# tnwei/waternet

Measured on NVIDIA H100. Metric: images/sec at 1080p batch16 (preprocess + gated-fusion forward, uint8 in -> uint8 out), higher is better.
Workload: dtype bf16 + fp8 corrections (v = hi + lo: hi x hi in bf16, both correction terms of the heavy layers as one e4m3 MMA; fp32 accumulate; 3-term bf16 elsewhere)

## Files before the change

### waternet_b200/csrc/umma_conv.cuh

```cuda
#pragma once

#include <cuda.h>
#include <cuda_bf16.h>

#include "common.cuh"
#include "wgmma_ops.cuh"

namespace wn {

__device__ __forceinline__ uint32_t smem_u32(const void* p) {
  return (uint32_t)__cvta_generic_to_shared(p);
}
__device__ __forceinline__ void mbar_init(uint64_t* bar, uint32_t count) {
  asm volatile("mbarrier.init.shared::cta.b64 [%0], %1;" ::"r"(smem_u32(bar)), "r"(count));
}
__device__ __forceinline__ void mbar_wait(uint64_t* bar, uint32_t parity) {
  for (uint32_t it = 0; it < (1u << 26); it++) {
    uint32_t done;
    asm volatile(
        "{\n\t.reg .pred p;\n\t"
        "mbarrier.try_wait.parity.shared::cta.b64 p, [%1], %2;\n\t"
        "selp.u32 %0, 1, 0, p;\n\t}"
        : "=r"(done)
        : "r"(smem_u32(bar)), "r"(parity)
        : "memory");
    if (done) return;
  }
  __trap();
}
__device__ __forceinline__ void mbar_arrive(uint64_t* bar) {
  asm volatile("mbarrier.arrive.shared::cta.b64 _, [%0];" ::"r"(smem_u32(bar)) : "memory");
}
__device__ __forceinline__ void mbar_expect_tx(uint64_t* bar, uint32_t bytes) {
  asm volatile("mbarrier.arrive.expect_tx.shared::cta.b64 _, [%0], %1;" ::"r"(smem_u32(bar)), "r"(bytes)
               : "memory");
}
__device__ __forceinline__ void tma_load_5d(void* dst, const CUtensorMap* tmap, uint64_t* bar, int c0,
                                            int c1, int c2, int c3, int c4) {
  asm volatile(
      "cp.async.bulk.tensor.5d.shared::cluster.global.mbarrier::complete_tx::bytes [%0], [%1, {%3, %4, %5, %6, %7}], [%2];"
      ::"r"(smem_u32(dst)), "l"(tmap), "r"(smem_u32(bar)), "r"(c0), "r"(c1), "r"(c2), "r"(c3), "r"(c4)
      : "memory");
}
__device__ __forceinline__ void bulk_load(void* dst, const void* src, uint32_t bytes, uint64_t* bar) {
  asm volatile(
      "cp.async.bulk.shared::cluster.global.mbarrier::complete_tx::bytes [%0], [%1], %2, [%3];" ::"r"(
          smem_u32(dst)),
      "l"(src), "r"(bytes), "r"(smem_u32(bar))
      : "memory");
}
__device__ __forceinline__ uint64_t make_desc(uint32_t addr, uint32_t lbo, uint32_t sbo) {
  return (uint64_t)((addr >> 4) & 0x3fff) | ((uint64_t)((lbo >> 4) & 0x3fff) << 16) |
         ((uint64_t)((sbo >> 4) & 0x3fff) << 32);
}
__device__ __forceinline__ void wg_fence() { asm volatile("wgmma.fence.sync.aligned;" ::: "memory"); }
__device__ __forceinline__ void wg_commit() { asm volatile("wgmma.commit_group.sync.aligned;" ::: "memory"); }
template <int PENDING>
__device__ __forceinline__ void wg_wait() { asm volatile("wgmma.wait_group.sync.aligned %0;" ::"n"(PENDING) : "memory"); }
__device__ __forceinline__ void wg_bar(int id) { asm volatile("bar.sync %0, 128;" ::"r"(id) : "memory"); }
__device__ __forceinline__ uint32_t pack_e4m3x4(float f0, float f1, float f2, float f3) {
  uint16_t lo, hi;
  asm("cvt.rn.satfinite.e4m3x2.f32 %0, %1, %2;" : "=h"(lo) : "f"(f1), "f"(f0));
  asm("cvt.rn.satfinite.e4m3x2.f32 %0, %1, %2;" : "=h"(hi) : "f"(f3), "f"(f2));
  return (uint32_t)lo | ((uint32_t)hi << 16);
}
__device__ __forceinline__ uint16_t pack_e4m3x2(float f0, float f1) {
  uint16_t v;
  asm("cvt.rn.satfinite.e4m3x2.f32 %0, %1, %2;" : "=h"(v) : "f"(f1), "f"(f0));
  return v;
}

enum Epilogue { kEpiAct = 0, kEpiSigmoid = 1, kEpiGate = 2, kEpiDgrad = 3 };

constexpr int kTileW = 8, kTileH = 16;
constexpr int kThreads = 320;
constexpr int kWarpA = 8, kWarpB = 9;
constexpr int kConsumerWarps = 8;
constexpr int kStageLd = 36;

constexpr int kFmtIn8 = 1, kFmtOut8 = 2;
template <int KS, int CIN_PAD, int NPAD, int CONCAT = 0, int NBLK = 1, int TPS = 1, int FMT = 0>
struct UmmaCfg {
  static constexpr bool F8IN = (FMT & kFmtIn8) != 0;
  static constexpr bool DUAL = CONCAT != 0;
  static constexpr int HALO_W = kTileW + KS - 1, HALO_H = kTileH + KS - 1;
  static constexpr int NCHUNK = CIN_PAD / 16;
  static constexpr int PLANE_BYTES = HALO_W * HALO_H * 16;
  static constexpr int A_STAGE = (4 * PLANE_BYTES + 1023) / 1024 * 1024;
  static constexpr int B_TAP = NPAD * 64;
  static constexpr int B_STAGE = TPS * B_TAP;
  static_assert((KS * KS) % TPS == 0, "taps per weight stage must divide the filter");
  static constexpr int NSTAGE_PER_CHUNK = KS * KS / TPS;
  static constexpr int STAGING = 2 * 64 * kStageLd * 4;
  static constexpr int BUDGET = 227 * 1024 - 1024 - 2048 - STAGING;
  static constexpr int NA_WANT = NCHUNK == 1 ? 2 : KS == 1 ? 6 : 3;
  static constexpr int NB_FIT = (BUDGET - NA_WANT * A_STAGE) / B_STAGE;
  static constexpr int NB = NB_FIT > 8 ? 8 : NB_FIT < 2 ? 2 : NB_FIT;
  static constexpr int NA_FIT = (BUDGET - NB * B_STAGE) / A_STAGE;
  static constexpr int NA = NA_FIT > NA_WANT ? NA_WANT : NA_FIT;
  static_assert(!F8IN || !CONCAT, "fp8 corrections: the [hi | second part] weight layout");
  static constexpr int CPB = NCHUNK / NBLK;
  static constexpr int BLK_COLS = DUAL ? 2 * NPAD : NPAD;
  static constexpr int COLS = NBLK * BLK_COLS;
  static constexpr int ACC = COLS / 2;
  static constexpr int ACC8 = F8IN ? ACC : 1;
  static constexpr int SMEM_BYTES = NA * A_STAGE + NB * B_STAGE + STAGING + 2048 + 1024;
  static_assert(NA >= 1, "halo tile does not fit in shared memory");
  static_assert(NCHUNK % NBLK == 0, "chunks must split evenly over the diagonal blocks");
  static_assert(NPAD % 16 == 0 && (DUAL ? 2 : 1) * NPAD <= 256, "invalid wgmma N");
  static_assert(ACC + (F8IN ? ACC8 : 0) <= 128, "accumulators do not fit in registers");
};

struct ActDst {
  uint4* base;
  int planes_half;
};

struct ConvArgs {
  const uint8_t* wpk;
  const float* bias;
  int N, H, W;
  int in_planes_half;
  int tiles_x, tiles_y;
  ActDst dst0, dst1;
  int split_c;
  int cout;
  float* out_f32;
  const float* cm;
  uint8_t* out_u8;
  const int* skip_lo;
  int a_hi_only;
  float* refined_out;
  const uint4* mask_base;
  int mask_planes_half;
  const float* f8_scale;
  int* f8_overflow;
  const int* run_if;
  int tiled;
  long long win0;
  TileGeom tiles;
  const RaggedWindow* rwin;
};

__device__ __forceinline__ uint32_t pack_bf16x2(__nv_bfloat16 a, __nv_bfloat16 b) {
  return (uint32_t)__bfloat16_as_ushort(a) | ((uint32_t)__bfloat16_as_ushort(b) << 16);
}
__device__ __forceinline__ void split_bf16x2(float f0, float f1, uint32_t& hi, uint32_t& lo) {
  const __nv_bfloat162 h = __floats2bfloat162_rn(f0, f1);
  hi = *reinterpret_cast<const uint32_t*>(&h);
  const float h0 = __uint_as_float(hi << 16), h1 = __uint_as_float(hi & 0xffff0000u);
  const __nv_bfloat162 l = __floats2bfloat162_rn(f0 - h0, f1 - h1);
  lo = *reinterpret_cast<const uint32_t*>(&l);
}

template <int EPI, bool OUT8, bool RAG = false>
__device__ __forceinline__ void epilogue16(const ConvArgs& g, const float* s_bias, const float* f, int ch, int n,
                                           int gx, int gy, bool valid = true) {
  const size_t hw = (size_t)g.H * g.W;
  const size_t pix = (size_t)gy * g.W + gx;
  if constexpr (EPI == kEpiAct || EPI == kEpiDgrad) {
    if (ch >= g.cout) return;
    if constexpr (OUT8) {
      uint32_t hi[8], l8[4], h8[4];
      float vmax = 0.f;
#pragma unroll
      for (int j = 0; j < 16; j += 4) {
        float v[4], r[4];
#pragma unroll
        for (int t = 0; t < 4; t++) {
          v[t] = fmaxf(f[j + t] + s_bias[ch + j + t], 0.f);
          if constexpr (RAG) v[t] = valid ? v[t] : 0.f;
          vmax = fmaxf(vmax, v[t]);
        }
#pragma unroll
        for (int t = 0; t < 4; t += 2) {
          const __nv_bfloat162 h = __floats2bfloat162_rn(v[t], v[t + 1]);
          const uint32_t hb = *reinterpret_cast<const uint32_t*>(&h);
          hi[(j + t) >> 1] = hb;
          r[t] = (v[t] - __uint_as_float(hb << 16)) * 512.f;
          r[t + 1] = (v[t + 1] - __uint_as_float(hb & 0xffff0000u)) * 512.f;
        }
        l8[j >> 2] = pack_e4m3x4(r[0], r[1], r[2], r[3]);
        h8[j >> 2] = pack_e4m3x4(v[0], v[1], v[2], v[3]);
      }
      if (!(vmax <= 448.f) && g.f8_overflow) atomicOr(g.f8_overflow, 1);
      const bool second = ch >= g.split_c;
      const ActDst& d = second ? g.dst1 : g.dst0;
      const int chl = second ? ch - g.split_c : ch;
      uint4* p_hi = d.base + ((size_t)n * 2 * d.planes_half + (chl >> 3)) * hw + pix;
      uint4* p_f8 = d.base + ((size_t)n * 2 * d.planes_half + d.planes_half + 2 * (chl >> 4)) * hw + pix;
      p_hi[0] = make_uint4(hi[0], hi[1], hi[2], hi[3]);
      p_hi[hw] = make_uint4(hi[4], hi[5], hi[6], hi[7]);
      p_f8[0] = make_uint4(l8[0], l8[1], l8[2], l8[3]);
      p_f8[hw] = make_uint4(h8[0], h8[1], h8[2], h8[3]);
    } else {
#pragma unroll
      for (int q = 0; q < 16; q += 8) {
        const int c = ch + q;
        if (c >= g.cout) break;
        uint32_t hi[4], lo[4];
        uint32_t mask[4] = {0xffffffffu, 0xffffffffu, 0xffffffffu, 0xffffffffu};
        if constexpr (EPI == kEpiDgrad) {
          if (g.mask_base) {
            const uint4 m = g.mask_base[((size_t)n * 2 * g.mask_planes_half + (c >> 3)) * hw + pix];
            mask[0] = m.x; mask[1] = m.y; mask[2] = m.z; mask[3] = m.w;
          }
        }
#pragma unroll
        for (int j = 0; j < 8; j += 2) {
          float f0, f1;
          if constexpr (EPI == kEpiDgrad) {
            f0 = (mask[j >> 1] & 0x0000ffffu) ? f[q + j] : 0.f;
            f1 = (mask[j >> 1] & 0xffff0000u) ? f[q + j + 1] : 0.f;
          } else {
            f0 = fmaxf(f[q + j] + s_bias[c + j], 0.f);
            f1 = fmaxf(f[q + j + 1] + s_bias[c + j + 1], 0.f);
            if constexpr (RAG) {
              f0 = valid ? f0 : 0.f;
              f1 = valid ? f1 : 0.f;
            }
          }
          split_bf16x2(f0, f1, hi[j >> 1], lo[j >> 1]);
        }
        const bool second = c >= g.split_c;
        const ActDst& d = second ? g.dst1 : g.dst0;
        const int plane = (second ? c - g.split_c : c) >> 3;
        uint4* p_hi = d.base + ((size_t)n * 2 * d.planes_half + plane) * hw + pix;
        p_hi[0] = make_uint4(hi[0], hi[1], hi[2], hi[3]);
        p_hi[(size_t)d.planes_half * hw] = make_uint4(lo[0], lo[1], lo[2], lo[3]);
      }
    }
  } else {
    if (ch != 0) return;
    const size_t o = (size_t)n * 3 * hw + pix;
    if constexpr (EPI == kEpiSigmoid) {
#pragma unroll
      for (int c = 0; c < 3; c++) g.out_f32[o + c * hw] = 1.0f / (1.0f + expf(-(f[c] + s_bias[c])));
    } else {
      float r[9];
#pragma unroll
      for (int j = 0; j < 9; j++) r[j] = fmaxf(f[j] + s_bias[j], 0.f);
      if (g.refined_out) {
#pragma unroll
        for (int j = 0; j < 9; j++) g.refined_out[(size_t)n * 9 * hw + pix + j * hw] = r[j];
      }
      if (g.cm) {
        const float c0 = g.cm[o], c1 = g.cm[o + hw], c2 = g.cm[o + 2 * hw];
        float v[3];
#pragma unroll
        for (int c = 0; c < 3; c++)
          v[c] = __fadd_rn(__fadd_rn(__fmul_rn(r[c], c0), __fmul_rn(r[3 + c], c1)), __fmul_rn(r[6 + c], c2));
        size_t oo = o, ohw = hw, o8 = ((size_t)n * hw + pix) * 3;
        float* out_f32 = g.out_f32;
        uint8_t* out_u8 = g.out_u8;
        if constexpr (RAG) {
          const RaggedWindow& t = g.rwin[n];
          const int y = t.ys + gy, x = t.xs + gx;
          if (y < t.ky0 || y >= t.ky1 || x < t.kx0 || x >= t.kx1) return;
          ohw = (size_t)t.H * t.W;
          oo = (size_t)y * t.W + x;
          o8 = oo * 3;
          out_f32 = t.out_f32;
          out_u8 = t.out_u8;
        } else if (g.tiled) {
          const TileWindow t = tile_window(g.tiles, g.win0 + n);
          const int y = t.ys + gy, x = t.xs + gx;
          if (y < t.ky0 || y >= t.ky1 || x < t.kx0 || x >= t.kx1) return;
          ohw = (size_t)g.tiles.H * g.tiles.W;
          const size_t ipix = (size_t)y * g.tiles.W + x;
          oo = (size_t)t.img * 3 * ohw + ipix;
          o8 = ((size_t)t.img * ohw + ipix) * 3;
        }
        if (out_f32) {
#pragma unroll
          for (int c = 0; c < 3; c++) out_f32[oo + c * ohw] = v[c];
        }
        if (out_u8) {
          uint8_t* q = out_u8 + o8;
#pragma unroll
          for (int c = 0; c < 3; c++) q[c] = (uint8_t)(int)__fmul_rn(fminf(fmaxf(v[c], 0.0f), 1.0f), 255.0f);
        }
      }
    }
  }
}

template <int KS, int CIN_PAD, int NPAD, int EPI, int CONCAT, int NBLK, int TPS, int FMT = 0, bool RAG = false>
__global__ void __launch_bounds__(kThreads, 1)
conv_umma_kernel(const __grid_constant__ CUtensorMap tmap_in, const ConvArgs g) {
  using C = UmmaCfg<KS, CIN_PAD, NPAD, CONCAT, NBLK, TPS, FMT>;
  constexpr bool F8IN = C::F8IN, DUAL = C::DUAL, OUT8 = (FMT & kFmtOut8) != 0;
  static_assert(!OUT8 || EPI == kEpiAct, "fp8 planes are written by the activation epilogue only");
  static_assert(!RAG || EPI == kEpiAct || EPI == kEpiGate, "ragged passes mask activations and store the gate");
  if (g.run_if != nullptr && *reinterpret_cast<const volatile int*>(g.run_if) == 0) return;
  extern __shared__ uint8_t smem_raw[];
  uint8_t* smem = reinterpret_cast<uint8_t*>((reinterpret_cast<uintptr_t>(smem_raw) + 1023) & ~(uintptr_t)1023);
  uint8_t* a_stages = smem;
  uint8_t* b_stages = smem + C::NA * C::A_STAGE;
  float* staging = reinterpret_cast<float*>(b_stages + C::NB * C::B_STAGE);
  uint8_t* tail = reinterpret_cast<uint8_t*>(staging) + C::STAGING;
  uint64_t* a_full = reinterpret_cast<uint64_t*>(tail);
  uint64_t* a_empty = a_full + C::NA;
  uint64_t* b_full = a_empty + C::NA;
  uint64_t* b_empty = b_full + C::NB;
  float* s_bias = reinterpret_cast<float*>(tail + 512);
  static_assert((2 * 6 + 2 * 8) * 8 <= 512 && NBLK * NPAD * 4 <= 2048 - 512, "barrier / bias area");

  const int tid = threadIdx.x, warp = tid >> 5, lane = tid & 31;
  const int num_tiles = g.tiles_x * g.tiles_y * g.N;
  if (tid == 0) {
    for (int i = 0; i < C::NA; i++) { mbar_init(&a_full[i], 1); mbar_init(&a_empty[i], kConsumerWarps); }
    for (int i = 0; i < C::NB; i++) { mbar_init(&b_full[i], 1); mbar_init(&b_empty[i], kConsumerWarps); }
    asm volatile("fence.mbarrier_init.release.cluster;" ::: "memory");
  }
  for (int i = tid; i < NBLK * NPAD; i += kThreads) s_bias[i] = g.bias[i];
  __syncthreads();

  if (warp == kWarpA) {
    if (lane == 0) {
      int stage = 0;
      uint32_t phase = 0;
      for (int tile = blockIdx.x; tile < num_tiles; tile += gridDim.x) {
        const int n = tile / (g.tiles_x * g.tiles_y);
        const int rem = tile - n * g.tiles_x * g.tiles_y;
        const int ty = rem / g.tiles_x, tx = rem - ty * g.tiles_x;
        const int x0 = tx * kTileW - KS / 2, y0 = ty * kTileH - KS / 2;
        for (int c = 0; c < C::NCHUNK; c++) {
          mbar_wait(&a_empty[stage], phase ^ 1);
          uint8_t* dst = a_stages + stage * C::A_STAGE;
          mbar_expect_tx(&a_full[stage], (g.a_hi_only ? 2 : 4) * C::PLANE_BYTES);
          tma_load_5d(dst, &tmap_in, &a_full[stage], 0, x0, y0, 2 * c, n);
          if (!g.a_hi_only)
            tma_load_5d(dst + 2 * C::PLANE_BYTES, &tmap_in, &a_full[stage], 0, x0, y0, g.in_planes_half + 2 * c, n);
          if (++stage == C::NA) { stage = 0; phase ^= 1; }
        }
      }
    }
    return;
  }
  if (warp == kWarpB) {
    if (lane == 0) {
      int stage = 0;
      uint32_t phase = 0;
      for (int tile = blockIdx.x; tile < num_tiles; tile += gridDim.x) {
        for (int it = 0; it < C::NCHUNK * C::NSTAGE_PER_CHUNK; it++) {
          mbar_wait(&b_empty[stage], phase ^ 1);
          mbar_expect_tx(&b_full[stage], C::B_STAGE);
          bulk_load(b_stages + stage * C::B_STAGE, g.wpk + (size_t)it * C::B_STAGE, C::B_STAGE, &b_full[stage]);
          if (++stage == C::NB) { stage = 0; phase ^= 1; }
        }
      }
    }
    return;
  }

  const int wg = warp >> 2, wtid = tid & 127;
  const bool skip_lo = (g.skip_lo != nullptr && *g.skip_lo != 0) || g.a_hi_only;
  const float dscale = F8IN ? *g.f8_scale : 1.f;
  constexpr uint32_t kSboA = C::HALO_W * 16;
  constexpr uint32_t kLboB = (CONCAT ? 2 * NPAD : NPAD) * 16;
  float acc[C::ACC], acc8[C::ACC8];
  int astage = 0, bstage = 0, pend_a = -1, pend_b = -1;
  uint32_t aphase = 0, bphase = 0;
  auto release = [&]() {
    if (lane == 0) {
      if (pend_b >= 0) mbar_arrive(&b_empty[pend_b]);
      if (pend_a >= 0) mbar_arrive(&a_empty[pend_a]);
    }
    pend_a = pend_b = -1;
  };
  for (int tile = blockIdx.x; tile < num_tiles; tile += gridDim.x) {
#pragma unroll
    for (int i = 0; i < C::ACC; i++) acc[i] = 0.f;
#pragma unroll
    for (int i = 0; i < C::ACC8; i++) acc8[i] = 0.f;
#pragma unroll
    for (int c = 0; c < C::NCHUNK; c++) {
      mbar_wait(&a_full[astage], aphase);
      const uint32_t a_base = smem_u32(a_stages + astage * C::A_STAGE) + (uint32_t)(wg * 8 * C::HALO_W * 16);
      const int blk = NBLK > 1 ? c / C::CPB : 0;
      for (int tg = 0; tg < C::NSTAGE_PER_CHUNK; tg++) {
        mbar_wait(&b_full[bstage], bphase);
        const uint32_t b_base = smem_u32(b_stages + bstage * C::B_STAGE);
        wg_fence();
#pragma unroll
        for (int t = 0; t < TPS; t++) {
          const int tap = tg * TPS + t;
          const int ky = tap / KS, kx = tap - ky * KS;
          const uint32_t a_tap = a_base + (uint32_t)((ky * C::HALO_W + kx) * 16);
          const uint32_t b_tap = b_base + (uint32_t)(t * C::B_TAP);
          const uint64_t a_hi = make_desc(a_tap, C::PLANE_BYTES, kSboA);
          const uint64_t a_lo = make_desc(a_tap + 2 * C::PLANE_BYTES, C::PLANE_BYTES, kSboA);
#pragma unroll
          for (int b = 0; b < NBLK; b++) {
            if (NBLK > 1 && b != blk) continue;
            float* d = acc + b * C::BLK_COLS / 2;
            if constexpr (F8IN) {
              wgmma_bf16<NPAD>(d, a_hi, make_desc(b_tap, NPAD * 16, 128));
              wgmma_e4m3<NPAD>(acc8 + b * C::BLK_COLS / 2, a_lo, make_desc(b_tap + NPAD * 32, NPAD * 16, 128));
            } else if constexpr (CONCAT) {
              wgmma_bf16<2 * NPAD>(d, a_hi, make_desc(b_tap, kLboB, 128));
              if (!skip_lo) wgmma_bf16<NPAD>(d, a_lo, make_desc(b_tap, kLboB, 128));
            } else {
              wgmma_bf16<NPAD>(d, a_hi, make_desc(b_tap, kLboB, 128));
              if (!skip_lo) wgmma_bf16<NPAD>(d, a_lo, make_desc(b_tap, kLboB, 128));
              wgmma_bf16<NPAD>(d, a_hi, make_desc(b_tap + 2 * NPAD * 16, kLboB, 128));
            }
          }
        }
        wg_commit();
        wg_wait<1>();
        release();
        pend_b = bstage;
        if (tg == C::NSTAGE_PER_CHUNK - 1) pend_a = astage;
        if (++bstage == C::NB) { bstage = 0; bphase ^= 1; }
      }
      if (++astage == C::NA) { astage = 0; aphase ^= 1; }
    }
    wg_wait<0>();
    release();

    const int n = tile / (g.tiles_x * g.tiles_y);
    const int rem = tile - n * g.tiles_x * g.tiles_y;
    const int ty = rem / g.tiles_x, tx = rem - ty * g.tiles_x;
    float* stg = staging + wg * 64 * kStageLd;
    const int frow = (warp & 3) * 16 + (lane >> 2), fcol = (lane & 3) * 2;
    const int r = wtid & 63, half = wtid >> 6;
    const int m = wg * 64 + r;
    const int gx = tx * kTileW + (m & 7), gy = ty * kTileH + (m >> 3);
    const bool inside = gx < g.W && gy < g.H;
    bool valid = true;
    if constexpr (RAG) valid = gx < g.rwin[n].vw && gy < g.rwin[n].vh;
    constexpr int NCH = NBLK * NPAD;
#pragma unroll
    for (int ch0 = 0; ch0 < NCH; ch0 += 32) {
#pragma unroll
      for (int j = 0; j < 4; j++) {
        const int ch = ch0 + 8 * j;
        if (ch < NCH) {
          const int col = NBLK > 1 ? (ch / NPAD) * C::BLK_COLS + ch % NPAD : ch;
          float v[4];
#pragma unroll
          for (int k = 0; k < 4; k++) {
            v[k] = acc[col / 2 + k];
            if constexpr (DUAL) v[k] += acc[(col + NPAD) / 2 + k];
            if constexpr (F8IN) v[k] = (v[k] + acc8[col / 2 + k]) * dscale;
          }
          float* s = stg + frow * kStageLd + 8 * j + fcol;
          *reinterpret_cast<float2*>(s) = make_float2(v[0], v[1]);
          *reinterpret_cast<float2*>(s + 8 * kStageLd) = make_float2(v[2], v[3]);
        }
      }
      wg_bar(1 + wg);
      const int cb = ch0 + 16 * half;
      if (cb < NCH && inside) {
        float f[16];
        const float4* s = reinterpret_cast<const float4*>(stg + r * kStageLd + 16 * half);
#pragma unroll
        for (int q = 0; q < 4; q++) {
          const float4 x = s[q];
          f[4 * q] = x.x; f[4 * q + 1] = x.y; f[4 * q + 2] = x.z; f[4 * q + 3] = x.w;
        }
        epilogue16<EPI, OUT8, RAG>(g, s_bias, f, cb, n, gx, gy, valid);
      }
      wg_bar(1 + wg);
    }
  }
}

static __global__ void scatter_weights_kernel(const float* __restrict__ src, float* __restrict__ dense, int co, int ci,
                                       int kk, int cinpad, int row_off, int split, int base0, int base1,
                                       float divisor) {
  const int total = co * ci * kk;
  for (int i = blockIdx.x * blockDim.x + threadIdx.x; i < total; i += gridDim.x * blockDim.x) {
    int t = i % kk;
    int c = (i / kk) % ci;
    int o = i / (kk * ci);
    int cd = c < split ? base0 + c : base1 + (c - split);
    dense[((size_t)(row_off + o) * cinpad + cd) * kk + t] = __fdiv_rn(src[i], divisor);
  }
}
static __global__ void scatter_bias_kernel(const float* __restrict__ src, float* __restrict__ dst, int co, int row_off) {
  for (int i = blockIdx.x * blockDim.x + threadIdx.x; i < co; i += gridDim.x * blockDim.x) dst[row_off + i] = src[i];
}
static __global__ void pack_stages_kernel(const float* __restrict__ dense, __nv_bfloat16* __restrict__ out, int npad,
                                   int cinpad, int kk, int concat, int nblk) {
  const int nchunk = cinpad / 16, cpb = nchunk / nblk;
  const size_t total = (size_t)nchunk * kk * 2 * 2 * npad * 8;
  for (size_t i = (size_t)blockIdx.x * blockDim.x + threadIdx.x; i < total; i += (size_t)gridDim.x * blockDim.x) {
    int e = (int)(i % 8);
    size_t r = i / 8;
    int k8, split, nrow;
    if (concat) {
      int row2 = (int)(r % (2 * npad)); r /= 2 * npad;
      k8 = (int)(r % 2); r /= 2;
      split = row2 >= npad;
      nrow = row2 - split * npad;
    } else {
      nrow = (int)(r % npad); r /= npad;
      k8 = (int)(r % 2); r /= 2;
      split = (int)(r % 2); r /= 2;
    }
    int tap = (int)(r % kk);
    int chunk = (int)(r / kk);
    int cin = chunk * 16 + k8 * 8 + e;
    int row = (chunk / cpb) * npad + nrow;
    float w = dense[((size_t)row * cinpad + cin) * kk + tap];
    __nv_bfloat16 hi = __float2bfloat16_rn(w);
    out[i] = split == 0 ? hi : __float2bfloat16_rn(w - __bfloat162float(hi));
  }
}


static __global__ void f8_absmax_kernel(const float* __restrict__ dense, size_t n, float* __restrict__ scale) {
  __shared__ float smax[256];
  float m = 0.f;
  for (size_t i = (size_t)blockIdx.x * blockDim.x + threadIdx.x; i < n; i += (size_t)gridDim.x * blockDim.x)
    m = fmaxf(m, fabsf(dense[i]));
  smax[threadIdx.x] = m;
  __syncthreads();
  for (int o = 128; o > 0; o >>= 1) {
    if ((int)threadIdx.x < o) smax[threadIdx.x] = fmaxf(smax[threadIdx.x], smax[threadIdx.x + o]);
    __syncthreads();
  }
  if (threadIdx.x == 0) atomicMax(reinterpret_cast<unsigned int*>(scale + 2), __float_as_uint(smax[0]));
}
static __global__ void f8_scale_finish_kernel(float* __restrict__ scale) {
  const float mx = fmaxf(scale[2], 1e-30f);
  const float ws = exp2f(floorf(log2f(224.f / mx)));
  scale[0] = ws;
  scale[1] = 1.f / (512.f * ws);
}
static __global__ void pack_stages_f8_kernel(const float* __restrict__ dense, uint8_t* __restrict__ out,
                                             const float* __restrict__ scale, int npad, int cinpad, int kk, int nblk) {
  const int nchunk = cinpad / 16, cpb = nchunk / nblk, rows = npad;
  const size_t tap_bytes = (size_t)rows * 64;
  const float ws = scale[0];
  const size_t total = (size_t)nchunk * kk * rows * 8;
  for (size_t i = (size_t)blockIdx.x * blockDim.x + threadIdx.x; i < total; i += (size_t)gridDim.x * blockDim.x) {
    size_t r = i;
    const int cp = (int)(r % 8); r /= 8;
    const int row = (int)(r % rows); r /= rows;
    const int tap = (int)(r % kk);
    const int chunk = (int)(r / kk);
    const int wrow = (chunk / cpb) * npad + row;
    float w[2], wl[2];
    uint16_t hb[2];
#pragma unroll
    for (int t = 0; t < 2; t++) {
      w[t] = dense[((size_t)wrow * cinpad + chunk * 16 + 2 * cp + t) * kk + tap];
      const __nv_bfloat16 h = __float2bfloat16_rn(w[t]);
      hb[t] = __bfloat16_as_ushort(h);
      wl[t] = w[t] - __bfloat162float(h);
    }
    uint8_t* base = out + ((size_t)chunk * kk + tap) * tap_bytes;
    const int c = 2 * cp;
#pragma unroll
    for (int t = 0; t < 2; t++)
      hb[t] = __bfloat16_as_ushort(__float2bfloat16_rn(__bfloat162float(__ushort_as_bfloat16(hb[t])) * ws * 512.f));
    *reinterpret_cast<uint32_t*>(base + ((size_t)(c / 8) * rows + row) * 16 + (c % 8) * 2) =
        (uint32_t)hb[0] | ((uint32_t)hb[1] << 16);
    uint8_t* p1 = base + (size_t)rows * 32;
    *reinterpret_cast<uint16_t*>(p1 + ((size_t)0 * rows + row) * 16 + c) = pack_e4m3x2(w[0] * ws, w[1] * ws);
    *reinterpret_cast<uint16_t*>(p1 + ((size_t)1 * rows + row) * 16 + c) =
        pack_e4m3x2(wl[0] * ws * 512.f, wl[1] * ws * 512.f);
  }
}

typedef CUresult (*EncodeTiledFn)(CUtensorMap*, CUtensorMapDataType, cuuint32_t, void*, const cuuint64_t*,
                                  const cuuint64_t*, const cuuint32_t*, const cuuint32_t*, CUtensorMapInterleave,
                                  CUtensorMapSwizzle, CUtensorMapL2promotion, CUtensorMapFloatOOBfill);
static EncodeTiledFn g_encode = nullptr;

static int get_encoder() {
  if (g_encode) return WN_OK;
  cudaDriverEntryPointQueryResult q;
  void* fn = nullptr;
  WN_CUDA(cudaGetDriverEntryPoint("cuTensorMapEncodeTiled", &fn, cudaEnableDefault, &q));
  if (!fn || q != cudaDriverEntryPointSuccess) {
    set_error("cuTensorMapEncodeTiled is not available from this driver");
    return WN_E_UNSUPPORTED;
  }
  g_encode = (EncodeTiledFn)fn;
  return WN_OK;
}

static int make_tmap(CUtensorMap* tm, void* base, int planes_total, int N, int H, int W, int halo_w, int halo_h) {
  cuuint64_t dims[5] = {8, (cuuint64_t)W, (cuuint64_t)H, (cuuint64_t)planes_total, (cuuint64_t)N};
  cuuint64_t strides[4] = {16, (cuuint64_t)W * 16, (cuuint64_t)H * W * 16, (cuuint64_t)planes_total * H * W * 16};
  cuuint32_t box[5] = {8, (cuuint32_t)halo_w, (cuuint32_t)halo_h, 2, 1};
  cuuint32_t estr[5] = {1, 1, 1, 1, 1};
  CUresult r = g_encode(tm, CU_TENSOR_MAP_DATA_TYPE_BFLOAT16, 5, base, dims, strides, box, estr,
                        CU_TENSOR_MAP_INTERLEAVE_NONE, CU_TENSOR_MAP_SWIZZLE_NONE, CU_TENSOR_MAP_L2_PROMOTION_L2_128B,
                        CU_TENSOR_MAP_FLOAT_OOB_FILL_NONE);
  if (r != CUDA_SUCCESS) {
    set_error("cuTensorMapEncodeTiled failed with %d (planes=%d N=%d H=%d W=%d box=%dx%d)", (int)r, planes_total, N, H,
              W, halo_w, halo_h);
    return WN_E_CUDA;
  }
  return WN_OK;
}

template <int KS, int CIN_PAD, int NPAD, int EPI, int CONCAT = 0, int NBLK = 1, int TPS = 1, int FMT = 0,
          bool RAG = false>
static int launch_conv(wn_handle* h, int slot, const uint8_t* wpk, const float* bias, void* in_base, ConvArgs a,
                       cudaStream_t stream) {
  using C = UmmaCfg<KS, CIN_PAD, NPAD, CONCAT, NBLK, TPS, FMT>;
  int rc = get_encoder();
  if (rc) return rc;
  CUtensorMap tm;
  rc = make_tmap(&tm, in_base, (a.a_hi_only ? 1 : 2) * (CIN_PAD / 8), a.N, a.H, a.W, C::HALO_W, C::HALO_H);
  if (rc) return rc;
  a.wpk = wpk;
  a.bias = bias;
  a.in_planes_half = CIN_PAD / 8;
  a.tiles_x = (a.W + kTileW - 1) / kTileW;
  a.tiles_y = (a.H + kTileH - 1) / kTileH;
  const long long tiles = (long long)a.tiles_x * a.tiles_y * a.N;
  auto kern = conv_umma_kernel<KS, CIN_PAD, NPAD, EPI, CONCAT, NBLK, TPS, FMT, RAG>;
  WN_CUDA(cudaFuncSetAttribute(kern, cudaFuncAttributeMaxDynamicSharedMemorySize, C::SMEM_BYTES));
  TimedScope ts(h, slot, stream);
  const int grid = (int)(tiles < h->sm_count ? tiles : h->sm_count);
  kern<<<grid, kThreads, C::SMEM_BYTES, stream>>>(tm, a);
  WN_LAUNCH_CHECK(h);
  return WN_OK;
}

}
```

Measured before the change: 48.75.

## Multicast weight stages across 2-CTA clusters to halve weight L2 traffic

The conv kernel now launches as 2-CTA clusters. Each CTA loads half of every weight stage and multicasts it to both CTAs, so each stage's weights are fetched once per pair rather than once per CTA. Weight-empty barriers now count arrivals from both CTAs' consumers through remote mbarrier arrives, and tiles are assigned in pairs. A CTA with no tile of its own still drains the weight stages. This adds cross-CTA coupling: the two CTAs must advance in lockstep through the weight pipeline, which can stall one on the other, and cluster occupancy limits may reduce the number of resident CTAs.

```diff
diff --git a/waternet_b200/csrc/umma_conv.cuh b/waternet_b200/csrc/umma_conv.cuh
--- a/waternet_b200/csrc/umma_conv.cuh
+++ b/waternet_b200/csrc/umma_conv.cuh
@@ -49,6 +49,39 @@
       "l"(src), "r"(bytes), "r"(smem_u32(bar))
       : "memory");
 }
+__device__ __forceinline__ void bulk_load_multicast(void* dst, const void* src, uint32_t bytes, uint64_t* bar,
+                                                    uint16_t cta_mask) {
+  asm volatile(
+      "cp.async.bulk.shared::cluster.global.mbarrier::complete_tx::bytes.multicast::cluster [%0], [%1], %2, [%3], %4;"
+      ::"r"(smem_u32(dst)), "l"(src), "r"(bytes), "r"(smem_u32(bar)), "h"(cta_mask)
+      : "memory");
+}
+__device__ __forceinline__ uint32_t cluster_ctarank() {
+  uint32_t r;
+  asm volatile("mov.u32 %0, %%cluster_ctarank;" : "=r"(r));
+  return r;
+}
+__device__ __forceinline__ uint32_t cluster_id_x() {
+  uint32_t r;
+  asm volatile("mov.u32 %0, %%clusterid.x;" : "=r"(r));
+  return r;
+}
+__device__ __forceinline__ uint32_t cluster_count_x() {
+  uint32_t r;
+  asm volatile("mov.u32 %0, %%nclusterid.x;" : "=r"(r));
+  return r;
+}
+__device__ __forceinline__ void cluster_sync() {
+  asm volatile("barrier.cluster.arrive.release.aligned;\n\tbarrier.cluster.wait.acquire.aligned;" ::: "memory");
+}
+__device__ __forceinline__ uint32_t mapa_shared(uint32_t addr, uint32_t rank) {
+  uint32_t r;
+  asm volatile("mapa.shared::cluster.u32 %0, %1, %2;" : "=r"(r) : "r"(addr), "r"(rank));
+  return r;
+}
+__device__ __forceinline__ void mbar_arrive_cluster(uint32_t cluster_addr) {
+  asm volatile("mbarrier.arrive.shared::cluster.b64 _, [%0];" ::"r"(cluster_addr) : "memory");
+}
 __device__ __forceinline__ uint64_t make_desc(uint32_t addr, uint32_t lbo, uint32_t sbo) {
   return (uint64_t)((addr >> 4) & 0x3fff) | ((uint64_t)((lbo >> 4) & 0x3fff) << 16) |
          ((uint64_t)((sbo >> 4) & 0x3fff) << 32);
@@ -76,6 +109,7 @@
 constexpr int kThreads = 320;
 constexpr int kWarpA = 8, kWarpB = 9;
 constexpr int kConsumerWarps = 8;
+constexpr int kClusterCtas = 2;
 constexpr int kStageLd = 36;
 
 constexpr int kFmtIn8 = 1, kFmtOut8 = 2;
@@ -89,6 +123,7 @@
   static constexpr int A_STAGE = (4 * PLANE_BYTES + 1023) / 1024 * 1024;
   static constexpr int B_TAP = NPAD * 64;
   static constexpr int B_STAGE = TPS * B_TAP;
+  static_assert((B_STAGE / kClusterCtas) % 16 == 0, "each CTA's share of a weight stage is a bulk copy (16 B units)");
   static_assert((KS * KS) % TPS == 0, "taps per weight stage must divide the filter");
   static constexpr int NSTAGE_PER_CHUNK = KS * KS / TPS;
   static constexpr int STAGING = 2 * 64 * kStageLd * 4;
@@ -286,7 +321,7 @@
 }
 
 template <int KS, int CIN_PAD, int NPAD, int EPI, int CONCAT, int NBLK, int TPS, int FMT = 0, bool RAG = false>
-__global__ void __launch_bounds__(kThreads, 1)
+__global__ void __cluster_dims__(kClusterCtas, 1, 1) __launch_bounds__(kThreads, 1)
 conv_umma_kernel(const __grid_constant__ CUtensorMap tmap_in, const ConvArgs g) {
   using C = UmmaCfg<KS, CIN_PAD, NPAD, CONCAT, NBLK, TPS, FMT>;
   constexpr bool F8IN = C::F8IN, DUAL = C::DUAL, OUT8 = (FMT & kFmtOut8) != 0;
@@ -308,19 +343,23 @@
 
   const int tid = threadIdx.x, warp = tid >> 5, lane = tid & 31;
   const int num_tiles = g.tiles_x * g.tiles_y * g.N;
+  const uint32_t rank = cluster_ctarank(), peer = rank ^ 1;
+  const int first_pair = (int)cluster_id_x(), pair_step = (int)cluster_count_x();
   if (tid == 0) {
     for (int i = 0; i < C::NA; i++) { mbar_init(&a_full[i], 1); mbar_init(&a_empty[i], kConsumerWarps); }
-    for (int i = 0; i < C::NB; i++) { mbar_init(&b_full[i], 1); mbar_init(&b_empty[i], kConsumerWarps); }
+    for (int i = 0; i < C::NB; i++) { mbar_init(&b_full[i], 1); mbar_init(&b_empty[i], kClusterCtas * kConsumerWarps); }
     asm volatile("fence.mbarrier_init.release.cluster;" ::: "memory");
   }
   for (int i = tid; i < NBLK * NPAD; i += kThreads) s_bias[i] = g.bias[i];
-  __syncthreads();
+  cluster_sync();
 
   if (warp == kWarpA) {
     if (lane == 0) {
       int stage = 0;
       uint32_t phase = 0;
-      for (int tile = blockIdx.x; tile < num_tiles; tile += gridDim.x) {
+      for (int j = first_pair; 2 * j < num_tiles; j += pair_step) {
+        const int tile = 2 * j + (int)rank;
+        if (tile >= num_tiles) continue;
         const int n = tile / (g.tiles_x * g.tiles_y);
         const int rem = tile - n * g.tiles_x * g.tiles_y;
         const int ty = rem / g.tiles_x, tx = rem - ty * g.tiles_x;
@@ -336,21 +375,28 @@
         }
       }
     }
+    __syncwarp();
+    cluster_sync();
     return;
   }
   if (warp == kWarpB) {
     if (lane == 0) {
+      constexpr uint32_t kHalf = C::B_STAGE / kClusterCtas;
       int stage = 0;
       uint32_t phase = 0;
-      for (int tile = blockIdx.x; tile < num_tiles; tile += gridDim.x) {
+      for (int j = first_pair; 2 * j < num_tiles; j += pair_step) {
         for (int it = 0; it < C::NCHUNK * C::NSTAGE_PER_CHUNK; it++) {
           mbar_wait(&b_empty[stage], phase ^ 1);
           mbar_expect_tx(&b_full[stage], C::B_STAGE);
-          bulk_load(b_stages + stage * C::B_STAGE, g.wpk + (size_t)it * C::B_STAGE, C::B_STAGE, &b_full[stage]);
+          bulk_load_multicast(b_stages + stage * C::B_STAGE + rank * kHalf,
+                              g.wpk + (size_t)it * C::B_STAGE + rank * kHalf, kHalf, &b_full[stage],
+                              (uint16_t)((1u << kClusterCtas) - 1));
           if (++stage == C::NB) { stage = 0; phase ^= 1; }
         }
       }
     }
+    __syncwarp();
+    cluster_sync();
     return;
   }
 
@@ -362,14 +408,28 @@
   float acc[C::ACC], acc8[C::ACC8];
   int astage = 0, bstage = 0, pend_a = -1, pend_b = -1;
   uint32_t aphase = 0, bphase = 0;
+  const uint32_t peer_b_empty = mapa_shared(smem_u32(b_empty), peer);
   auto release = [&]() {
     if (lane == 0) {
-      if (pend_b >= 0) mbar_arrive(&b_empty[pend_b]);
+      if (pend_b >= 0) {
+        mbar_arrive(&b_empty[pend_b]);
+        mbar_arrive_cluster(peer_b_empty + pend_b * (uint32_t)sizeof(uint64_t));
+      }
       if (pend_a >= 0) mbar_arrive(&a_empty[pend_a]);
     }
     pend_a = pend_b = -1;
   };
-  for (int tile = blockIdx.x; tile < num_tiles; tile += gridDim.x) {
+  for (int j = first_pair; 2 * j < num_tiles; j += pair_step) {
+    const int tile = 2 * j + (int)rank;
+    if (tile >= num_tiles) {
+      for (int it = 0; it < C::NCHUNK * C::NSTAGE_PER_CHUNK; it++) {
+        mbar_wait(&b_full[bstage], bphase);
+        pend_b = bstage;
+        release();
+        if (++bstage == C::NB) { bstage = 0; bphase ^= 1; }
+      }
+      continue;
+    }
 #pragma unroll
     for (int i = 0; i < C::ACC; i++) acc[i] = 0.f;
 #pragma unroll
@@ -466,6 +526,8 @@
       wg_bar(1 + wg);
     }
   }
+  __syncwarp();
+  cluster_sync();
 }
 
 static __global__ void scatter_weights_kernel(const float* __restrict__ src, float* __restrict__ dense, int co, int ci,
@@ -599,6 +661,26 @@
     return WN_E_CUDA;
   }
   return WN_OK;
+}
+
+template <typename Kernel>
+static int max_active_clusters(Kernel kern, int dev, int smem_bytes) {
+  constexpr int kMaxDevices = 64;
+  static int cached[kMaxDevices] = {};
+  if (dev >= 0 && dev < kMaxDevices && cached[dev] > 0) return cached[dev];
+  cudaLaunchConfig_t cfg = {};
+  cfg.gridDim = dim3(kClusterCtas);
+  cfg.blockDim = dim3(kThreads);
+  cfg.dynamicSmemBytes = smem_bytes;
+  int n = 0;
+  const cudaError_t err = cudaOccupancyMaxActiveClusters(&n, kern, &cfg);
+  if (err != cudaSuccess || n <= 0) {
+    set_error("no cluster of %d CTAs x %d threads with %d B of shared memory fits on device %d (%s)", kClusterCtas,
+              kThreads, smem_bytes, dev, cudaGetErrorString(err));
+    return 0;
+  }
+  if (dev >= 0 && dev < kMaxDevices) cached[dev] = n;
+  return n;
 }
 
 template <int KS, int CIN_PAD, int NPAD, int EPI, int CONCAT = 0, int NBLK = 1, int TPS = 1, int FMT = 0,
@@ -619,8 +701,11 @@
   const long long tiles = (long long)a.tiles_x * a.tiles_y * a.N;
   auto kern = conv_umma_kernel<KS, CIN_PAD, NPAD, EPI, CONCAT, NBLK, TPS, FMT, RAG>;
   WN_CUDA(cudaFuncSetAttribute(kern, cudaFuncAttributeMaxDynamicSharedMemorySize, C::SMEM_BYTES));
+  const int clusters = max_active_clusters(kern, h->device, C::SMEM_BYTES);
+  if (clusters == 0) return WN_E_UNSUPPORTED;
+  const long long pairs = (tiles + kClusterCtas - 1) / kClusterCtas;
   TimedScope ts(h, slot, stream);
-  const int grid = (int)(tiles < h->sm_count ? tiles : h->sm_count);
+  const int grid = kClusterCtas * (int)(pairs < clusters ? pairs : clusters);
   kern<<<grid, kThreads, C::SMEM_BYTES, stream>>>(tm, a);
   WN_LAUNCH_CHECK(h);
   return WN_OK;
```

New measurement: 49.35, median of 6. +1.2%, better.
